# integritychain/fips204

Measured on AMD Instinct MI355X. Metric: ML-DSA-65 verifies/sec per GPU (batched); % HBM roofline, higher is better.
Workload: dtype int32; 1 GPU; ml_dsa_65 batch=65536 whole verify on FIPS 204 wire formats; batch_per_gpu=65536, parallelism=batch-split x1

## Files before the change

### fips204_amd/vfy/vfy.hip

```cpp
#include <hip/hip_runtime.h>
#include <stdint.h>
#include <string.h>

#include <mutex>
#include <string>
#include <vector>

#include "../../include/mldsa_vfy.h"
#include "../layer/layer_dev.h"
#include "../layer/layer_host.h"
#include "../csrc/challenge_dev.h"
#include "../csrc/ntt_wave.h"
#include "../csrc/sampler_dev.h"
#include "../csrc/tables.h"
#include "../csrc/verify_dev.h"
#include "keccak180.h"
#include "vfy_parts.h"

namespace mldsa_vfy {

using mldsa::FWD_TW;
using mldsa::INV_TW;
using mldsa::N;
using mldsa::SHAKE256_RATE;
using mldsa::SWAVES;
using mldsa::Twiddle;
using mldsa::load_le32;
using mldsa::static_for;

#ifndef MLDSA_VFY_EA_WAVES
#define MLDSA_VFY_EA_WAVES 5
#endif
template <int K, int L>
__global__ __launch_bounds__(64 * SWAVES) __attribute__((amdgpu_waves_per_eu(MLDSA_VFY_EA_WAVES, MLDSA_VFY_EA_WAVES))) void k_expand_a(const uint8_t* __restrict__ rho, size_t rho_stride,
                                                                                                    const uint32_t* __restrict__ key_idx,
                                                                                                    int32_t* __restrict__ a_hat, size_t n_ops,
                                                                                                    uint32_t n_keys) {
    const int lane = threadIdx.x & 63;
    const size_t g = (size_t)blockIdx.x * (64 * SWAVES) + threadIdx.x;
    const size_t wave_base = g - lane;
    const size_t n_streams = n_ops * (size_t)(K * L);
    const bool valid = g < n_streams;
    const size_t op = valid ? g / (K * L) : 0;
    const int rs = valid ? (int)(g % (K * L)) : 0;
    const int r = rs / L, sidx = rs % L;
    KeccakState st;
    size_t key = key_idx ? key_idx[op] : op;
    if (n_keys && key >= n_keys) key = 0;
    mldsa::expand_a_seed(st, rho + key * rho_stride, sidx, r);
    rej_ntt_poly_lane_direct180(st, a_hat, wave_base, lane, valid);
}

__global__ __launch_bounds__(256) void k_unpack_a(const uint32_t* __restrict__ packed, int32_t* __restrict__ out, size_t n_polys) {
    const size_t poly = (size_t)blockIdx.x * 4 + (threadIdx.x >> 6);
    if (poly >= n_polys) return;
    const int lane = threadIdx.x & 63;
    const uint32_t* p = packed + poly * mldsa::PACKED_POLY_DWORDS + 3 * lane;
    reinterpret_cast<int4*>(out + poly * N)[lane] = mldsa::unpack24(mldsa::Packed3{p[0], p[1], p[2]});
}

__global__ __launch_bounds__(256) void k_sanitize_keys(const uint32_t* __restrict__ key_idx, uint32_t n_keys, size_t n_ops,
                                                       uint32_t* __restrict__ safe, int32_t* __restrict__ bad) {
    const size_t i = (size_t)blockIdx.x * 256 + threadIdx.x;
    if (i >= n_ops) return;
    const uint32_t k = key_idx[i];
    safe[i] = k < n_keys ? k : 0u;
    bad[i] = k < n_keys ? 0 : 2;
}

constexpr int MU_BLK_STRIDE = 35;
__global__ __launch_bounds__(64) void k_mu(const uint8_t* __restrict__ tr, size_t tr_stride, const uint32_t* __restrict__ key_idx, int mode,
                                           const uint8_t* __restrict__ msgs, const uint64_t* __restrict__ msg_off,
                                           const uint8_t* __restrict__ ctxs, const uint64_t* __restrict__ ctx_off, uint8_t* __restrict__ mu,
                                           size_t mu_stride, int32_t* __restrict__ ctx_bad, const int32_t* __restrict__ key_bad, size_t n_ops,
                                           size_t op0, size_t n_call) {
    __shared__ uint32_t blk[64 * MU_BLK_STRIDE];
    const int lane = threadIdx.x;
    const size_t op = (size_t)blockIdx.x * 64 + lane;
    const bool valid = op < n_ops;
    uint32_t* row = blk + lane * MU_BLK_STRIDE;
    uint8_t* rowb = reinterpret_cast<uint8_t*>(row);

    const uint8_t *trp = nullptr, *mp = nullptr, *cp = nullptr;
    size_t mlen = 0, clen = 0;
    bool live = false;
    if (valid) {
        trp = tr + (key_idx ? key_idx[op] : op) * tr_stride;
        const uint64_t m0 = msg_off[op0 + op], m1 = msg_off[op0 + op + 1];
        bool bad_off = !(msg_off[0] <= m0 && m0 <= m1 && m1 <= msg_off[n_call]);
        mp = msgs + m0;
        mlen = (size_t)(m1 - m0);
        bad_off |= mlen != 0 && msgs == nullptr;
        if (ctx_off) {
            const uint64_t c0 = ctx_off[op0 + op], c1 = ctx_off[op0 + op + 1];
            bad_off |= !(ctx_off[0] <= c0 && c0 <= c1 && c1 <= ctx_off[n_call]);
            cp = ctxs + c0;
            clen = (size_t)(c1 - c0);
            bad_off |= clen != 0 && ctxs == nullptr;
        }
        const int flag = bad_off ? 2 : clen > 255 ? 1 : (key_bad ? key_bad[op] : 0);
        ctx_bad[op] = flag;
        live = !bad_off && clen <= 255;
        if (!live) mlen = clen = 0;
    }
    const size_t pre = (mode == MLDSA_MODE_INTERNAL) ? 0 : 2 + clen;
    const size_t total = live ? 64 + pre + mlen : 0;
    const size_t my_blocks = live ? total / SHAKE256_RATE + 1 : 0;
    size_t max_blocks = my_blocks;
#pragma unroll
    for (int m = 32; m >= 1; m >>= 1) {
        const size_t o = (size_t)__shfl_xor((unsigned long long)max_blocks, m);
        max_blocks = o > max_blocks ? o : max_blocks;
    }
    KeccakState st;
    mldsa::keccak_zero(st);
    for (size_t b = 0; b < max_blocks; b++) {
        if (b < my_blocks) {
            const size_t base = b * SHAKE256_RATE;
            auto byte_at = [&](size_t pos) -> uint8_t {
                if (pos < total) {
                    if (pos < 64) return trp[pos];
                    if (pos < 64 + pre) {
                        const size_t q = pos - 64;
                        return q == 0 ? (uint8_t)(mode == MLDSA_MODE_PREHASH ? 1 : 0) : q == 1 ? (uint8_t)clen : cp[q - 2];
                    }
                    return mp[pos - 64 - pre];
                }
                return pos == total ? (uint8_t)0x1F : (uint8_t)0;
            };
            for (int i = 0; i < SHAKE256_RATE / 4; i++) {
                const size_t pos = base + 4 * (size_t)i;
                uint32_t v;
                if (pos + 4 <= 64) v = load_le32(trp + pos);
                else if (pos >= 64 + pre && pos + 4 <= total) v = load_le32(mp + (pos - 64 - pre));
                else if (pos > total) v = 0;
                else v = (uint32_t)byte_at(pos) | ((uint32_t)byte_at(pos + 1) << 8) | ((uint32_t)byte_at(pos + 2) << 16) | ((uint32_t)byte_at(pos + 3) << 24);
                row[i] = v;
            }
            if (b == my_blocks - 1) rowb[SHAKE256_RATE - 1] |= 0x80;
            static_for<0, 17>([&](auto wc) {
                constexpr int W = decltype(wc)::value;
                st.lo[W] ^= row[2 * W];
                st.hi[W] ^= row[2 * W + 1];
            });
            mldsa::keccak_f1600(st);
        }
    }
    if (valid) {
        uint32_t* out = reinterpret_cast<uint32_t*>(mu + op * mu_stride);
#pragma unroll
        for (int i = 0; i < 8; i++) {
            out[2 * i] = st.lo[i];
            out[2 * i + 1] = st.hi[i];
        }
    }
}

template <int CT>
__global__ __launch_bounds__(64) void k_sample_in_ball(const uint8_t* __restrict__ c_tilde, size_t ct_stride, int tau, uint32_t* __restrict__ c_out,
                                                       size_t n_ops) {
    __shared__ uint32_t c_lds[64 * mldsa::SIB_C_STRIDE];
    __shared__ uint32_t b_lds[64 * mldsa::SIB_BLK_STRIDE];
    const int lane = threadIdx.x;
    const size_t wave_base = (size_t)blockIdx.x * 64;
    const size_t op = wave_base + lane;
    const bool valid = op < n_ops;
    KeccakState st;
    mldsa::keccak_zero(st);
    if (valid) mldsa::absorb_words<CT / 8>(st, c_tilde + op * ct_stride);
    mldsa::shake_pad<SHAKE256_RATE, CT>(st);
    mldsa::sample_in_ball_lane(st, tau, valid, c_lds + lane * mldsa::SIB_C_STRIDE, b_lds + lane * mldsa::SIB_BLK_STRIDE);
    mldsa::wave_lds_sync();
    for (int row = 0; row < 64; row++) {
        if (wave_base + row >= n_ops) break;
        const uint8_t* cb = reinterpret_cast<const uint8_t*>(c_lds + row * mldsa::SIB_C_STRIDE);
        c_out[(wave_base + row) * 64 + lane] =
            (uint32_t)cb[lane] | ((uint32_t)cb[64 + lane] << 8) | ((uint32_t)cb[128 + lane] << 16) | ((uint32_t)cb[192 + lane] << 24);
    }
}

template <int CTRL>
__device__ __forceinline__ int32_t dpp_all(int32_t v) {
    return __builtin_amdgcn_update_dpp(0, v, CTRL, 0xF, 0xF, true);
}

template <int M>
__device__ __forceinline__ void swap_pair(int32_t& x, int32_t& y, int lane) {
    if constexpr (M >= 4) {
        mldsa::swap_pair<M>(x, y, lane);
    } else {
        constexpr int CTRL = M == 2 ? 0x4E : 0xB1;
        const int32_t px = dpp_all<CTRL>(x), py = dpp_all<CTRL>(y);
        const bool up = (lane & M) != 0;
        x = up ? py : x;
        y = up ? y : px;
    }
}
template <int M>
__device__ __forceinline__ void xchg_hi(int32_t r[4], int lane) {
    swap_pair<M>(r[0], r[2], lane);
    swap_pair<M>(r[1], r[3], lane);
}
template <int M>
__device__ __forceinline__ void xchg_lo(int32_t r[4], int lane) {
    swap_pair<M>(r[0], r[1], lane);
    swap_pair<M>(r[2], r[3], lane);
}

template <class TW>
__device__ __forceinline__ void ntt_fwd_wave(int32_t r[4], const TW& tw, int lane) {
    using mldsa::bf_ct;
    bf_ct(r[0], r[2], mldsa::ZF1);
    bf_ct(r[1], r[3], mldsa::ZF1);
    bf_ct(r[0], r[1], mldsa::ZF2);
    bf_ct(r[2], r[3], mldsa::ZF3);
    xchg_hi<32>(r, lane);
    bf_ct(r[0], r[2], tw.get(0));
    bf_ct(r[1], r[3], tw.get(1));
    xchg_lo<16>(r, lane);
    bf_ct(r[0], r[1], tw.get(2));
    bf_ct(r[2], r[3], tw.get(3));
    xchg_hi<8>(r, lane);
    bf_ct(r[0], r[2], tw.get(4));
    bf_ct(r[1], r[3], tw.get(5));
    xchg_lo<4>(r, lane);
    bf_ct(r[0], r[1], tw.get(6));
    bf_ct(r[2], r[3], tw.get(7));
    xchg_hi<2>(r, lane);
    bf_ct(r[0], r[2], tw.get(8));
    bf_ct(r[1], r[3], tw.get(9));
    xchg_lo<1>(r, lane);
    bf_ct(r[0], r[1], tw.get(10));
    bf_ct(r[2], r[3], tw.get(11));
}
template <class TW>
__device__ __forceinline__ void ntt_inv_wave(int32_t r[4], const TW& tw, int lane, int32_t f) {
    using mldsa::bf_gs;
    bf_gs(r[0], r[1], tw.get(0));
    bf_gs(r[2], r[3], tw.get(1));
    bf_gs(r[0], r[2], tw.get(2));
    bf_gs(r[1], r[3], tw.get(3));
    xchg_lo<1>(r, lane);
    bf_gs(r[0], r[1], tw.get(4));
    bf_gs(r[2], r[3], tw.get(5));
    xchg_hi<2>(r, lane);
    bf_gs(r[0], r[2], tw.get(6));
    bf_gs(r[1], r[3], tw.get(7));
    xchg_lo<4>(r, lane);
    bf_gs(r[0], r[1], tw.get(8));
    bf_gs(r[2], r[3], tw.get(9));
    xchg_hi<8>(r, lane);
    bf_gs(r[0], r[2], tw.get(10));
    bf_gs(r[1], r[3], tw.get(11));
    xchg_lo<16>(r, lane);
    bf_gs(r[0], r[1], tw.get(12));
    bf_gs(r[2], r[3], tw.get(13));
    xchg_hi<32>(r, lane);
    const int32_t zf = (int32_t)((((int64_t)mldsa::ZI1 * f) % mldsa::Q) * mldsa::RINV_MOD_Q % mldsa::Q);
#pragma unroll
    for (int k = 0; k < 2; k++) {
        const int32_t a = r[k], b = r[k + 2];
        r[k] = mldsa::caddq(mldsa::mont_mul(a + b, f));
        r[k + 2] = mldsa::caddq(mldsa::mont_mul(a - b, zf));
    }
}

template <bool G2HI>
__device__ __forceinline__ void pack_w1_strided(const uint32_t v[4], uint8_t* dst, int lane) {
    if constexpr (G2HI) {
        uint32_t d[4];
#pragma unroll
        for (int k = 0; k < 4; k++) d[k] = v[k] << (4 * (lane & 7));
#pragma unroll
        for (int k = 0; k < 4; k++) d[k] |= (uint32_t)dpp_all<0xB1>((int32_t)d[k]);
#pragma unroll
        for (int k = 0; k < 4; k++) d[k] |= (uint32_t)dpp_all<0x4E>((int32_t)d[k]);
        const uint32_t d01 = (lane & 1) ? d[1] : d[0], d23 = (lane & 1) ? d[3] : d[2];
        uint32_t mine = (lane & 2) ? d23 : d01;
        mine |= (uint32_t)__builtin_amdgcn_update_dpp(0, (int32_t)mine, 0x104, 0xF, 0xF, true);
        if (!(lane & 4)) mldsa::store_row(reinterpret_cast<uint32_t*>(dst) + 8 * (lane & 3) + (lane >> 3), mine);
    } else {
#pragma unroll
        for (int k = 0; k < 4; k++) {
            const uint32_t n1 = (uint32_t)dpp_all<0xB1>((int32_t)v[k]);
            const uint32_t pair = (lane & 1) ? 0u : (v[k] | (n1 << 6));
            const uint32_t n2 = (uint32_t)dpp_all<0x4E>((int32_t)pair);
            if (!(lane & 3)) {
                const uint32_t q24 = pair | (n2 << 12);
                uint8_t* d = dst + 48 * k + 3 * (lane >> 2);
                d[0] = (uint8_t)q24; d[1] = (uint8_t)(q24 >> 8); d[2] = (uint8_t)(q24 >> 16);
            }
        }
    }
}

constexpr int VW = 4;
template <int K, int L, int GB, bool G2HI, int MINW>
__global__ __launch_bounds__(64 * VW) __attribute__((amdgpu_waves_per_eu(MINW))) void k_verify_main(
    const uint32_t* __restrict__ a_hat, const uint8_t* __restrict__ sigs, size_t sig_len, int ctilde_len, const uint32_t* __restrict__ c,
    const int32_t* __restrict__ t1, const uint32_t* __restrict__ key_idx, size_t key_base, int32_t* __restrict__ hvalid, int omega,
    uint8_t* __restrict__ w1, size_t w1_stride, int32_t* __restrict__ znorm, int32_t zbound, size_t n_ops, const Twiddle* __restrict__ fwd_tab,
    const Twiddle* __restrict__ inv_tab) {
    using mldsa::Packed3;
    constexpr int CB = GB + 1;
    constexpr int BITS = G2HI ? 4 : 6;
    __shared__ int4 zh[VW][L + 1][64];
    __shared__ uint32_t hint_lds[VW][mldsa::HINT_LDS_DWORDS];
    __shared__ Twiddle tw_lds[(FWD_TW + INV_TW) * 64];
    const int lane = threadIdx.x & 63;
    const int wave = __builtin_amdgcn_readfirstlane(threadIdx.x >> 6);
    for (int i = threadIdx.x; i < FWD_TW * 64; i += 64 * VW) tw_lds[i] = fwd_tab[i];
    for (int i = threadIdx.x; i < INV_TW * 64; i += 64 * VW) tw_lds[FWD_TW * 64 + i] = inv_tab[i];
    __syncthreads();
    const mldsa::LdsTw ftw{tw_lds, lane};
    const mldsa::LdsTw itw{tw_lds + FWD_TW * 64, lane};
    const uint32_t wid = blockIdx.x * VW + wave, n_waves = gridDim.x * VW;

    for (size_t op = wid; op < n_ops; op += n_waves) {
        unsigned ul = (unsigned)lane;
        asm volatile("" : "+v"(ul));
        const size_t key = key_idx ? (size_t)__builtin_amdgcn_readfirstlane((int)key_idx[op]) : key_base + op;
        const Packed3* arow = reinterpret_cast<const Packed3*>(a_hat + (op * K * (size_t)L) * mldsa::PACKED_POLY_DWORDS);
        const int4* trow = reinterpret_cast<const int4*>(t1 + (key * K) * (size_t)N);
        Packed3 av[L];
#pragma unroll
        for (int j = 0; j < L; j++) av[j] = mldsa::load_row<mldsa::NT_A_VERIFY>(&arow[(unsigned)(j * 64) + ul]);
        int4 tv = trow[ul];
        const uint8_t* zsrc = sigs + op * sig_len + ctilde_len;
        const mldsa::HintBytes hbytes = mldsa::hint_load(zsrc + L * (32 * CB), omega, K, (int)ul);
        bool zbad = false;
#pragma unroll 1
        for (int j = 0; j <= L; j++) {
            asm volatile("" ::: "memory");
            int32_t r[4];
            if (j < L) {
                const uint8_t* src = zsrc + (size_t)j * (32 * CB);
                int32_t mx = 0;
#pragma unroll
                for (int k = 0; k < 4; k++) {
                    r[k] = mldsa::y_from_raw<CB>(mldsa::y_raw_dword<CB, mldsa::NT_ZC>(src, k, (int)ul), (int)ul);
                    const int32_t a = r[k] < 0 ? -r[k] : r[k];
                    mx = a > mx ? a : mx;
                }
                zbad |= mx >= zbound;
            } else {
                const uint32_t d = mldsa::load_once<mldsa::NT_ZC>(c + op * 64 + ul);
                r[0] = (int8_t)(d & 0xFF); r[1] = (int8_t)((d >> 8) & 0xFF); r[2] = (int8_t)((d >> 16) & 0xFF); r[3] = (int8_t)(d >> 24);
            }
            mldsa_vfy::ntt_fwd_wave(r, ftw, lane);
            if (j == L) {
#pragma unroll
                for (int k = 0; k < 4; k++) r[k] = mldsa::mont_mul(r[k], -1);
            }
            zh[wave][j][lane] = make_int4(r[0], r[1], r[2], r[3]);
        }
        const bool hint_ok = mldsa::hint_unpack_wave<K>(hbytes, omega, hint_lds[wave], (int)ul);
        if (lane == 0) {
            znorm[op] = __ballot(zbad) != 0ull ? 0x7fffffff : 0;
            hvalid[op] = hint_ok ? 1 : 0;
        }
        auto row = [&](int i, const Packed3 (&a_cur)[L], const int4& t_cur, Packed3 (&a_nxt)[L], int4& t_nxt, bool more) {
            const int4 cv = zh[wave][L][lane];
            int64_t acc64[4] = {(int64_t)cv.x * t_cur.x, (int64_t)cv.y * t_cur.y, (int64_t)cv.z * t_cur.z, (int64_t)cv.w * t_cur.w};
#pragma unroll
            for (int j = 0; j < L; j++) {
                const int4 zv = zh[wave][j][lane];
                const int4 a4 = mldsa::unpack24(a_cur[j]);
                acc64[0] += (int64_t)a4.x * zv.x;
                acc64[1] += (int64_t)a4.y * zv.y;
                acc64[2] += (int64_t)a4.z * zv.z;
                acc64[3] += (int64_t)a4.w * zv.w;
            }
            int32_t acc[4];
            if (more) {
#pragma unroll
                for (int j = 0; j < L; j++) a_nxt[j] = mldsa::load_row<mldsa::NT_A_VERIFY>(&arow[(unsigned)(((i + 1) * L + j) * 64) + ul]);
                t_nxt = trow[(unsigned)((i + 1) * 64) + ul];
            }
#pragma unroll
            for (int k = 0; k < 4; k++) acc[k] = mldsa::mont_reduce64(acc64[k]);
            mldsa_vfy::ntt_inv_wave(acc, itw, lane, mldsa::F_MONT2);
            const uint32_t* hrow = hint_lds[wave] + 24 + i * 8 + (ul >> 5);
            uint8_t* dst = w1 + op * w1_stride + (size_t)i * (32 * BITS);
            uint32_t v[4];
#pragma unroll
            for (int k = 0; k < 4; k++) {
                const uint32_t h = (hrow[2 * k] >> (ul & 31)) & 1u;
                v[k] = (uint32_t)mldsa::use_hint<G2HI>((int32_t)h, acc[k]);
            }
            pack_w1_strided<G2HI>(v, dst, lane);
        };
        static_assert(K % 2 == 0, "the row loop runs two rows a trip");
        Packed3 aw[L];
        int4 tw2;
#pragma unroll 1
        for (int i = 0; i < K; i += 2) {
            asm volatile("" ::: "memory");
            row(i, av, tv, aw, tw2, true);
            asm volatile("" ::: "memory");
            row(i + 1, aw, tw2, av, tv, i + 2 < K);
        }
    }
}

constexpr int CWAVES = 4;
constexpr int CBLOCK = 64 * CWAVES;
template <int OUT>
__global__ __launch_bounds__(CBLOCK) void k_ctilde_verdict(const uint8_t* __restrict__ mu_w1, size_t mw, const uint8_t* __restrict__ sigs, size_t sig_len,
                                                           const int32_t* __restrict__ znorm, int32_t zbound, const int32_t* __restrict__ hvalid,
                                                           const int32_t* __restrict__ ctx_bad, uint8_t* __restrict__ ok, size_t n_ops) {
    __shared__ uint32_t tiles[CWAVES * 64 * mldsa::H_STRIDE];
    __shared__ unsigned long long ptr_a[CWAVES * 64];
    const int lane = threadIdx.x & 63, wave = threadIdx.x >> 6;
    uint32_t* tile = tiles + wave * 64 * mldsa::H_STRIDE;
    const size_t base_op = (size_t)blockIdx.x * CBLOCK;
    if (base_op >= n_ops) return;
    const size_t op = base_op + threadIdx.x;
    const bool valid = op < n_ops;
    const size_t opc = valid ? op : base_op;
    ptr_a[wave * 64 + lane] = (unsigned long long)(mu_w1 + opc * mw);
    mldsa::wave_lds_sync_c();
    KeccakState st;
    mldsa::shake256_2_absorb<true>(st, tile, ptr_a + wave * 64, ptr_a + wave * 64, (int)mw, 0, 0, 0, lane);
    if (!valid) return;
    const uint8_t* c0 = sigs + op * sig_len;
    uint32_t diff = 0;
    static_for<0, OUT / 8>([&](auto wc) {
        constexpr int W = decltype(wc)::value;
        diff |= (st.lo[W] ^ load_le32(c0 + 8 * W)) | (st.hi[W] ^ load_le32(c0 + 8 * W + 4));
    });
    ok[op] = (uint8_t)(diff == 0 && znorm[op] < zbound && hvalid[op] && !ctx_bad[op]);
}

}

namespace {

using namespace mldsa_layer;
using namespace mldsa_vfy;

struct DevState {
    int dev = -1;
    int n_cu = 256;
    hipStream_t ea = nullptr, vm = nullptr;
    std::vector<hipEvent_t> ev;
    Twiddle *fwd = nullptr, *inv = nullptr;
    bool prof_on = false;
    std::vector<hipEvent_t> prof_ev;
    std::vector<const char*> prof_name;
    size_t prof_used = 0;
};

std::mutex g_mutex;
std::vector<DevState*> g_states;
size_t g_part_ops = 0;

size_t part_ops() { return g_part_ops ? g_part_ops : (size_t)MLDSA_VFY_PART_OPS; }

int dev_state(const char* fn, int dev, DevState** out) {
    for (DevState* d : g_states)
        if (d->dev == dev) {
            *out = d;
            return MLDSA_OK;
        }
    DevState* d = new DevState;
    d->dev = dev;
    int cu = 0;
    if (hipDeviceGetAttribute(&cu, hipDeviceAttributeMultiprocessorCount, dev) == hipSuccess && cu > 0) d->n_cu = cu;
    const std::vector<mldsa::HostTwiddle> f = mldsa::gen_fwd_lane_twiddles(), i = mldsa::gen_inv_lane_twiddles();
    hipError_t e = hipStreamCreateWithFlags(&d->ea, hipStreamNonBlocking);
    if (e == hipSuccess) e = hipStreamCreateWithFlags(&d->vm, hipStreamNonBlocking);
    if (e == hipSuccess) e = hipMalloc(&d->fwd, f.size() * sizeof(Twiddle));
    if (e == hipSuccess) e = hipMalloc(&d->inv, i.size() * sizeof(Twiddle));
    if (e == hipSuccess) e = hipMemcpy(d->fwd, f.data(), f.size() * sizeof(Twiddle), hipMemcpyHostToDevice);
    if (e == hipSuccess) e = hipMemcpy(d->inv, i.data(), i.size() * sizeof(Twiddle), hipMemcpyHostToDevice);
    if (e != hipSuccess || f.size() != (size_t)FWD_TW * 64 || i.size() != (size_t)INV_TW * 64) {
        if (d->ea) (void)hipStreamDestroy(d->ea);
        if (d->vm) (void)hipStreamDestroy(d->vm);
        if (d->fwd) (void)hipFree(d->fwd);
        if (d->inv) (void)hipFree(d->inv);
        delete d;
        (void)hipGetLastError();
        return e != hipSuccess ? hip_failed(fn, "creating the library's streams and tables", e)
                               : fail(MLDSA_ERR_DEVICE, std::string(fn) + ": the core's twiddle tables have another shape");
    }
    g_states.push_back(d);
    *out = d;
    return MLDSA_OK;
}

struct Events {
    DevState* d;
    size_t used = 0;
    hipError_t err = hipSuccess;
    explicit Events(DevState* d_) : d(d_) {}
    hipEvent_t next() {
        if (used == d->ev.size()) {
            hipEvent_t e = nullptr;
            const hipError_t rc = hipEventCreateWithFlags(&e, hipEventDisableTiming);
            if (rc != hipSuccess) {
                err = rc;
                return nullptr;
            }
            d->ev.push_back(e);
        }
        return d->ev[used++];
    }
};

constexpr size_t PROF_MAX_PAIRS = 4096;
struct ProfScope {
    DevState* d;
    hipStream_t s;
    long idx = -1;
    ProfScope(DevState* d_, hipStream_t s_, const char* name) : d(d_), s(s_) {
        if (!d->prof_on || d->prof_used >= PROF_MAX_PAIRS) return;
        if (d->prof_used * 2 + 2 > d->prof_ev.size()) {
            hipEvent_t a = nullptr, b = nullptr;
            if (hipEventCreate(&a) != hipSuccess) return;
            if (hipEventCreate(&b) != hipSuccess) {
                (void)hipEventDestroy(a);
                return;
            }
            d->prof_ev.push_back(a);
            d->prof_ev.push_back(b);
            d->prof_name.push_back(name);
        } else {
            d->prof_name[d->prof_used] = name;
        }
        idx = (long)d->prof_used++;
        (void)hipEventRecord(d->prof_ev[2 * idx], s);
    }
    ~ProfScope() {
        if (idx >= 0) (void)hipEventRecord(d->prof_ev[2 * idx + 1], s);
    }
};

#define VFY_HIP(call, what)                                     \
    do {                                                        \
        const hipError_t e_ = (call);                           \
        if (e_ != hipSuccess) return hip_failed(fn, what, e_);  \
    } while (0)

#define VFY_BY_SET(set, M)              \
    do {                                \
        if ((set) == MLDSA_44) M(4, 4, 17, false, 32, 5); \
        else if ((set) == MLDSA_65) M(6, 5, 19, true, 48, 4); \
        else M(8, 7, 19, true, 64, 4);  \
    } while (0)

unsigned stream_blocks(size_t n_streams) { return (unsigned)((n_streams + 64 * SWAVES - 1) / (64 * SWAVES)); }

void launch_expand_a(int set, const uint8_t* rho, const uint32_t* key_idx, int32_t* a_hat, size_t n, uint32_t n_keys, hipStream_t s) {
    mldsa_params p;
    (void)mldsa_get_params(set, &p);
    const dim3 grid(stream_blocks(n * (size_t)(p.k * p.l))), block(64 * SWAVES);
#define VFY_EA(KK, LL, GB, G2, CT, MW) hipLaunchKernelGGL((k_expand_a<KK, LL>), grid, block, 0, s, rho, (size_t)32, key_idx, a_hat, n, n_keys)
    VFY_BY_SET(set, VFY_EA);
#undef VFY_EA
}

struct Call {
    int set, mode;
    mldsa_params p;
    const uint8_t *rho, *tr;
    const int32_t* t1;
    size_t n_keys;
    const uint32_t* key_idx;
    const uint8_t* msgs;
    const uint64_t* msg_off;
    const uint8_t* ctxs;
    const uint64_t* ctx_off;
    const uint8_t* sigs;
    uint8_t* ok;
    size_t n_ops;
};

int enqueue(const char* fn, DevState* d, const Call& c, uint8_t* scratch, hipStream_t s) {
    const mldsa_params& p = c.p;
    const PartPlan plan(c.n_ops, part_ops());
    const Carve cv = carve(p.k, p.l, (size_t)p.w1_len, plan);
    const size_t mw = 64 + (size_t)p.w1_len;
    uint32_t* c8 = reinterpret_cast<uint32_t*>(scratch + cv.c);
    int32_t* znorm = reinterpret_cast<int32_t*>(scratch + cv.znorm);
    int32_t* hvalid = reinterpret_cast<int32_t*>(scratch + cv.hvalid);
    int32_t* ctx_bad = reinterpret_cast<int32_t*>(scratch + cv.ctx_bad);
    int32_t* key_bad = reinterpret_cast<int32_t*>(scratch + cv.key_bad);
    uint32_t* kidx = reinterpret_cast<uint32_t*>(scratch + cv.kidx);
    uint8_t* mu_w1 = scratch + cv.mu_w1;
    const size_t sig_len = (size_t)p.sig_len;

    const OrderPlan order = order_plan(plan.n_parts());
    const hipStream_t lanes[N_LANES] = {s, d->ea, d->vm};
    Events evs(d);
    std::vector<hipEvent_t> ev(order.n_events);
    for (hipEvent_t& e : ev) e = evs.next();
    if (evs.err != hipSuccess) return hip_failed(fn, "creating an event", evs.err);

    for (const Step& st : order.steps) {
        const hipStream_t q = lanes[st.lane];
        if (st.act == ACT_RECORD) {
            VFY_HIP(hipEventRecord(ev[st.n], q), (std::string("recording ") + st.what).c_str());
            continue;
        }
        if (st.act == ACT_WAIT) {
            VFY_HIP(hipStreamWaitEvent(q, ev[st.n], 0), (std::string("waiting for ") + st.what).c_str());
            continue;
        }
        const Part part = plan.at(st.n);
        const size_t o = part.first, n = part.count;
        const size_t key_base = c.key_idx ? 0 : o;
        int32_t* a_hat = reinterpret_cast<int32_t*>(scratch + cv.ring[part.half]);
        const uint8_t* sg = c.sigs + o * sig_len;
        const uint32_t* kp = c.key_idx ? kidx + o : nullptr;
        const int32_t* kb = c.key_idx ? key_bad + o : nullptr;
        switch (st.stage) {
        case STAGE_EXPAND_A: {
            ProfScope ps(d, q, "expand_a");
            launch_expand_a(c.set, c.rho + key_base * 32, c.key_idx ? c.key_idx + o : nullptr, a_hat, n, c.key_idx ? (uint32_t)c.n_keys : 0u, q);
            break;
        }
        case STAGE_FRONT: {
            if (c.key_idx)
                hipLaunchKernelGGL(k_sanitize_keys, dim3((unsigned)((n + 255) / 256)), dim3(256), 0, q, c.key_idx + o, (uint32_t)c.n_keys, n, kidx + o, key_bad + o);
            {
                ProfScope ps(d, q, "mu");
                hipLaunchKernelGGL(k_mu, dim3((unsigned)((n + 63) / 64)), dim3(64), 0, q, c.tr + key_base * 64, (size_t)64, kp, c.mode, c.msgs, c.msg_off, c.ctxs,
                                   c.ctx_off, mu_w1 + o * mw, mw, ctx_bad + o, kb, n, o, c.n_ops);
            }
            {
                ProfScope ps(d, q, "sample_in_ball");
                const dim3 grid((unsigned)((n + 63) / 64)), block(64);
#define VFY_SIB(KK, LL, GB, G2, CT, MW) hipLaunchKernelGGL((k_sample_in_ball<CT>), grid, block, 0, q, sg, sig_len, p.tau, c8 + o * 64, n)
                VFY_BY_SET(c.set, VFY_SIB);
#undef VFY_SIB
            }
            break;
        }
        case STAGE_VERIFY_MAIN: {
            ProfScope ps(d, q, "verify_main");
            const size_t need = (n + VW - 1) / VW, cap = (size_t)d->n_cu * 16;
            const dim3 grid((unsigned)(need < cap ? need : cap)), block(64 * VW);
#define VFY_VM(KK, LL, GB, G2, CT, MW)                                                                                                         \
    hipLaunchKernelGGL((k_verify_main<KK, LL, GB, G2, MW>), grid, block, 0, q, reinterpret_cast<const uint32_t*>(a_hat), sg, sig_len,          \
                       p.ctilde_len, c8 + o * 64, c.t1, kp, key_base, hvalid + o, p.omega, mu_w1 + o * mw + 64, mw, znorm + o, p.gamma1 - p.beta, n, \
                       d->fwd, d->inv)
            VFY_BY_SET(c.set, VFY_VM);
#undef VFY_VM
            break;
        }
        default: {
            ProfScope ps(d, q, "ctilde_hash");
            const dim3 grid((unsigned)((n + CBLOCK - 1) / CBLOCK)), block(CBLOCK);
#define VFY_CT(KK, LL, GB, G2, CT, MW)                                                                                                    \
    hipLaunchKernelGGL((k_ctilde_verdict<CT>), grid, block, 0, q, mu_w1 + o * mw, mw, sg, sig_len, znorm + o, p.gamma1 - p.beta, hvalid + o, \
                       ctx_bad + o, c.ok + o, n)
            VFY_BY_SET(c.set, VFY_CT);
#undef VFY_CT
            break;
        }
        }
        LAYER_LAUNCHED(st.what);
    }
    return MLDSA_OK;
}

void drain(DevState* d) {
    (void)hipStreamSynchronize(d->ea);
    (void)hipStreamSynchronize(d->vm);
    (void)hipGetLastError();
}

size_t scratch_bytes_of(int set, size_t n_ops) {
    mldsa_params p;
    if (mldsa_get_params(set, &p) != MLDSA_OK || n_ops > MLDSA_VFY_MAX_OPS) return 0;
    return carve(p.k, p.l, (size_t)p.w1_len, PartPlan(n_ops, part_ops())).bytes;
}

}

extern "C" {

int mldsa_vfy_abi_version(void) { return MLDSA_VFY_ABI_VERSION; }

const char* mldsa_vfy_last_error(void) { return g_err.c_str(); }

size_t mldsa_vfy_scratch_bytes(int set, size_t n_ops) {
    std::lock_guard<std::mutex> lk(g_mutex);
    return scratch_bytes_of(set, n_ops);
}

size_t mldsa_vfy_set_part_ops(size_t part) {
    std::lock_guard<std::mutex> lk(g_mutex);
    const size_t before = part_ops();
    g_part_ops = part;
    return before;
}

int mldsa_vfy_verify(mldsa_ctx* ctx, int set, int mode, const uint8_t* rho, const uint8_t* tr, const int32_t* t1_d2_hat_mont, size_t n_keys,
                     const uint32_t* key_idx, const uint8_t* msgs, const uint64_t* msg_off, const uint8_t* ctxs, const uint64_t* ctx_off,
                     const uint8_t* sigs, uint8_t* ok, size_t n_ops, void* scratch, size_t scratch_bytes, void* stream) {
    const char* fn = "mldsa_vfy_verify";
    Call c;
    const int rc = check_common(fn, ctx, set, n_ops, MLDSA_VFY_MAX_OPS, "MLDSA_VFY_MAX_OPS ops", &c.p);
    if (rc != MLDSA_OK) return rc;
    if (mode != MLDSA_MODE_PURE && mode != MLDSA_MODE_INTERNAL && mode != MLDSA_MODE_PREHASH)
        return fail(MLDSA_ERR_PARAM, std::string(fn) + ": bad mode");
    if (n_ops == 0) return MLDSA_OK;
    if (!rho || !tr || !t1_d2_hat_mont || !msg_off || !sigs || !ok) return fail(MLDSA_ERR_PARAM, std::string(fn) + ": NULL pointer");
    if (key_idx ? n_keys == 0 : n_keys < n_ops) return fail(MLDSA_ERR_PARAM, std::string(fn) + ": n_keys does not cover the batch");
    if (n_keys > 0xFFFFFFFFu) n_keys = 0xFFFFFFFFu;
    if (!aligned(t1_d2_hat_mont, 16)) return fail(MLDSA_ERR_PARAM, std::string(fn) + ": t1_d2_hat_mont must be 16-byte aligned");
    if (!scratch || !aligned(scratch, 256)) return fail(MLDSA_ERR_PARAM, std::string(fn) + ": scratch is NULL or not 256-byte aligned");
    LAYER_ON_DEVICE(ctx);
    std::lock_guard<std::mutex> lk(g_mutex);
    if (scratch_bytes < scratch_bytes_of(set, n_ops))
        return fail(MLDSA_ERR_NOMEM, std::string(fn) + ": scratch is below mldsa_vfy_scratch_bytes(set, n_ops)");
    DevState* d = nullptr;
    const int src = dev_state(fn, dev_, &d);
    if (src != MLDSA_OK) return src;
    c.set = set; c.mode = mode; c.rho = rho; c.tr = tr; c.t1 = t1_d2_hat_mont; c.n_keys = n_keys; c.key_idx = key_idx; c.msgs = msgs;
    c.msg_off = msg_off; c.ctxs = ctxs; c.ctx_off = ctx_off; c.sigs = sigs; c.ok = ok; c.n_ops = n_ops;
    const int erc = enqueue(fn, d, c, static_cast<uint8_t*>(scratch), (hipStream_t)stream);
    if (erc != MLDSA_OK) drain(d);
    return erc;
}

int mldsa_vfy_expand_a(mldsa_ctx* ctx, int set, const uint8_t* rho, int32_t* a_hat, size_t n_ops, void* stream) {
    const char* fn = "mldsa_vfy_expand_a";
    mldsa_params p;
    const int rc = check_common(fn, ctx, set, n_ops, MLDSA_VFY_MAX_OPS, "MLDSA_VFY_MAX_OPS ops", &p);
    if (rc != MLDSA_OK) return rc;
    if (n_ops == 0) return MLDSA_OK;
    if (!rho || !a_hat) return fail(MLDSA_ERR_PARAM, std::string(fn) + ": NULL pointer");
    if (!aligned(a_hat, 16)) return fail(MLDSA_ERR_PARAM, std::string(fn) + ": a_hat must be 16-byte aligned");
    LAYER_ON_DEVICE(ctx);
    hipStream_t s = (hipStream_t)stream;
    const size_t n_polys = n_ops * (size_t)(p.k * p.l);
    void* packed = nullptr;
    VFY_HIP(hipMalloc(&packed, n_polys * PACKED_POLY_BYTES), "allocating the packed rows");
    launch_expand_a(set, rho, nullptr, static_cast<int32_t*>(packed), n_ops, 0u, s);
    hipLaunchKernelGGL(k_unpack_a, dim3((unsigned)((n_polys + 3) / 4)), dim3(256), 0, s, static_cast<const uint32_t*>(packed), a_hat, n_polys);
    hipError_t e = hipGetLastError();
    const hipError_t se = hipStreamSynchronize(s);
    if (e == hipSuccess) e = se;
    (void)hipFree(packed);
    return e == hipSuccess ? MLDSA_OK : hip_failed(fn, "ExpandA and unpack", e);
}

int mldsa_vfy_profile_enable(mldsa_ctx* ctx, int on) {
    const char* fn = "mldsa_vfy_profile_enable";
    if (!ctx) return fail(MLDSA_ERR_PARAM, std::string(fn) + ": NULL context");
    LAYER_ON_DEVICE(ctx);
    std::lock_guard<std::mutex> lk(g_mutex);
    DevState* d = nullptr;
    const int rc = dev_state(fn, dev_, &d);
    if (rc != MLDSA_OK) return rc;
    d->prof_on = on != 0;
    if (!d->prof_on) d->prof_used = 0;
    return MLDSA_OK;
}

int mldsa_vfy_profile_report(mldsa_ctx* ctx, char* buf, size_t buf_len) {
    const char* fn = "mldsa_vfy_profile_report";
    if (!ctx) return fail(MLDSA_ERR_PARAM, std::string(fn) + ": NULL context");
    if (!buf || buf_len <= 2) return fail(MLDSA_ERR_PARAM, std::string(fn) + ": bad argument");
    LAYER_ON_DEVICE(ctx);
    std::lock_guard<std::mutex> lk(g_mutex);
    DevState* d = nullptr;
    const int rc = dev_state(fn, dev_, &d);
    if (rc != MLDSA_OK) return rc;
    VFY_HIP(hipDeviceSynchronize(), "waiting for the device");
    struct Acc { const char* name; double ms; size_t calls; };
    std::vector<Acc> acc;
    for (size_t i = 0; i < d->prof_used; i++) {
        float ms = 0.f;
        if (hipEventElapsedTime(&ms, d->prof_ev[2 * i], d->prof_ev[2 * i + 1]) != hipSuccess) {
            (void)hipGetLastError();
            continue;
        }
        bool found = false;
        for (auto& a : acc)
            if (strcmp(a.name, d->prof_name[i]) == 0) {
                a.ms += ms;
                a.calls++;
                found = true;
                break;
            }
        if (!found) acc.push_back({d->prof_name[i], ms, 1});
    }
    std::string out = "{";
    for (size_t i = 0; i < acc.size(); i++)
        out += std::string(i ? ", " : "") + "\"" + acc[i].name + "\": {\"ms\": " + std::to_string(acc[i].ms) + ", \"calls\": " + std::to_string(acc[i].calls) + "}";
    out += "}";
    if (out.size() + 1 > buf_len) return fail(MLDSA_ERR_PARAM, std::string(fn) + ": buffer too small");
    memcpy(buf, out.c_str(), out.size() + 1);
    d->prof_used = 0;
    return MLDSA_OK;
}

}
```

### fips204_amd/vfy/vfy_parts.h

```cpp
#pragma once
#include <stddef.h>
#include <stdint.h>

#include <vector>

namespace mldsa_vfy {

constexpr size_t PACKED_POLY_BYTES = 768;
constexpr size_t CARVE_ALIGN = 256;

struct Part {
    size_t first = 0, count = 0;
    int half = 0;
};

struct PartPlan {
    size_t n_ops, part;
    PartPlan(size_t n_ops_, size_t part_) : n_ops(n_ops_), part(part_ ? part_ : 1) {}
    size_t n_parts() const { return n_ops / part + (n_ops % part ? 1 : 0); }
    size_t halves() const { return n_parts() > 1 ? 2 : n_parts(); }
    size_t half_ops() const { return n_ops < part ? n_ops : part; }
    Part at(size_t i) const {
        Part p;
        p.first = i * part;
        p.count = n_ops - p.first < part ? n_ops - p.first : part;
        p.half = (int)(i & 1);
        return p;
    }
};

struct Carve {
    size_t ring[2];
    size_t ring_bytes;
    size_t c;
    size_t znorm, hvalid, ctx_bad, key_bad, kidx;
    size_t mu_w1;
    size_t bytes;
};

inline size_t carve_up(size_t x) { return (x + CARVE_ALIGN - 1) / CARVE_ALIGN * CARVE_ALIGN; }

inline Carve carve(int k, int l, size_t w1_len, const PartPlan& plan) {
    Carve c;
    size_t at = 0;
    auto take = [&at](size_t bytes) {
        const size_t here = at;
        at += carve_up(bytes);
        return here;
    };
    c.ring_bytes = plan.half_ops() * (size_t)(k * l) * PACKED_POLY_BYTES;
    c.ring[0] = take(c.ring_bytes);
    c.ring[1] = plan.halves() > 1 ? take(c.ring_bytes) : c.ring[0];
    c.c = take(plan.n_ops * 256);
    c.znorm = take(plan.n_ops * 4);
    c.hvalid = take(plan.n_ops * 4);
    c.ctx_bad = take(plan.n_ops * 4);
    c.key_bad = take(plan.n_ops * 4);
    c.kidx = take(plan.n_ops * 4);
    c.mu_w1 = take(plan.n_ops * (64 + w1_len));
    c.bytes = at + CARVE_ALIGN;
    return c;
}

enum Lane { LANE_CALLER = 0, LANE_EA = 1, LANE_VM = 2, N_LANES = 3 };
enum Action { ACT_RECORD, ACT_WAIT, ACT_LAUNCH };
enum Stage { STAGE_EXPAND_A = 0, STAGE_FRONT = 1, STAGE_VERIFY_MAIN = 2, STAGE_CTILDE = 3, N_STAGES = 4 };

struct Step {
    Lane lane;
    Action act;
    Stage stage;
    size_t n;
    const char* what;
};

struct OrderPlan {
    std::vector<Step> steps;
    size_t n_events = 0;
};

struct StageLanes {
    Lane expand_a, arith, front;
};
inline StageLanes lanes_of_call(size_t n_parts) {
    return n_parts == 1 ? StageLanes{LANE_CALLER, LANE_CALLER, LANE_VM} : StageLanes{LANE_EA, LANE_VM, LANE_CALLER};
}

inline OrderPlan order_plan(size_t n_parts, const StageLanes& on) {
    OrderPlan o;
    if (n_parts == 0) return o;
    const size_t none = (size_t)-1;
    auto put = [&o](Lane lane, Action act, Stage stage, size_t n, const char* what) { o.steps.push_back(Step{lane, act, stage, n, what}); };
    const size_t fork = o.n_events++;
    bool forked[N_LANES] = {true, false, false};
    auto reach = [&](Lane lane, Stage stage) {
        if (!forked[lane]) put(lane, ACT_WAIT, stage, fork, "the fork");
        forked[lane] = true;
    };
    auto record = [&](Lane from, Lane to, Stage stage, const char* what) {
        if (from == to) return none;
        put(from, ACT_RECORD, stage, o.n_events, what);
        return o.n_events++;
    };
    auto wait = [&](Lane to, size_t event, Stage stage, const char* what) {
        if (event == none) return;
        put(to, ACT_WAIT, stage, event, what);
        forked[to] = true;
    };
    put(LANE_CALLER, ACT_RECORD, STAGE_EXPAND_A, fork, "the fork");
    std::vector<size_t> used(n_parts, none);
    for (size_t p = 0; p < n_parts; p++) {
        if (p >= 2) wait(on.expand_a, used[p - 2], STAGE_EXPAND_A, "the ring half");
        reach(on.expand_a, STAGE_EXPAND_A);
        put(on.expand_a, ACT_LAUNCH, STAGE_EXPAND_A, p, "k_expand_a launch");
        const size_t ready = record(on.expand_a, on.arith, STAGE_EXPAND_A, "ExpandA's end");
        reach(on.front, STAGE_FRONT);
        put(on.front, ACT_LAUNCH, STAGE_FRONT, p, "front launch");
        const size_t front = record(on.front, on.arith, STAGE_FRONT, "the front's end");
        wait(on.arith, ready, STAGE_EXPAND_A, "ExpandA");
        wait(on.arith, front, STAGE_FRONT, "the front");
        reach(on.arith, STAGE_VERIFY_MAIN);
        put(on.arith, ACT_LAUNCH, STAGE_VERIFY_MAIN, p, "k_verify_main launch");
        if (p + 2 < n_parts) used[p] = record(on.arith, on.expand_a, STAGE_VERIFY_MAIN, "the end of the ring half's use");
        put(on.arith, ACT_LAUNCH, STAGE_CTILDE, p, "k_ctilde_verdict launch");
    }
    wait(LANE_CALLER, record(on.arith, LANE_CALLER, STAGE_CTILDE, "the join"), STAGE_CTILDE, "the join");
    return o;
}

inline OrderPlan order_plan(size_t n_parts) { return order_plan(n_parts, lanes_of_call(n_parts)); }

}
```

Measured before the change: 41.16 million verifies/s.

## Batch forward NTTs of z and c across lane groups with register butterflies

Replaces the serial per-polynomial forward NTT loop (one poly per wave pass, 4 coefficients per lane) with passes that process 4 or 2 polynomials at once. Each lane holds 16 or 8 coefficients, so the early NTT levels run as in-register butterflies with compile-time zetas and only the later levels use cross-lane swaps and a 256-entry zeta table. The LDS row is padded to 65 entries to avoid bank conflicts on the new store pattern, and the forward twiddle table is loaded only when a leftover single pass still needs it. The intent is fewer cross-lane exchanges and fewer serialized passes per op, at the cost of higher register pressure and more code, which may reduce occupancy.

Result: no change. 41.33 million verifies/s, median of 6 (+0.4%).

```diff
diff --git a/fips204_amd/vfy/vfy.hip b/fips204_amd/vfy/vfy.hip
--- a/fips204_amd/vfy/vfy.hip
+++ b/fips204_amd/vfy/vfy.hip
@@ -265,6 +265,78 @@
     }
 }
 
+constexpr int ZH_ROW = 65;
+template <int P>
+constexpr FwdPlan FWD_PLAN = fwd_plan(P);
+template <int P, int J0, int CB, int L>
+__device__ __forceinline__ bool fwd_pass(const uint8_t* zsrc, const uint32_t* c_op, int4 (*zw)[ZH_ROW], const Twiddle* zt, int32_t zbound, unsigned ul) {
+    using mldsa::bf_ct;
+    constexpr int R = 4 * P, W = 64 / P;
+    static_assert(J0 + P <= L + 1 && (W * CB) % 8 == 0, "the slots are polynomials of the op; a register's fields start at whole bytes");
+    constexpr bool HAS_C = J0 + P == L + 1;
+    constexpr int LP = FWD_PLAN<P>.lp, RB = FWD_PLAN<P>.rb;
+    const unsigned p = ul & (P - 1), l = ul >> LP;
+    const bool is_c = HAS_C && p == P - 1;
+    int32_t r[R];
+    bool zbad = false;
+    if (!is_c) {
+        const uint8_t* src = zsrc + (size_t)(J0 + p) * (32 * CB);
+        int32_t mx = 0;
+#pragma unroll
+        for (int k = 0; k < R; k++) {
+            r[k] = mldsa::y_from_raw<CB>(mldsa::y_raw_dword<CB, mldsa::NT_ZC>(src + k * (W * CB / 8), 0, (int)l), (int)l);
+            const int32_t a = r[k] < 0 ? -r[k] : r[k];
+            mx = a > mx ? a : mx;
+        }
+        zbad = mx >= zbound;
+    } else {
+        uint32_t d[P];
+#pragma unroll
+        for (int q = 0; q < P; q++) d[q] = mldsa::load_once<mldsa::NT_ZC>(c_op + W * q + l);
+#pragma unroll
+        for (int k = 0; k < R; k++) r[k] = (int8_t)((d[k % P] >> (8 * (k / P))) & 0xFF);
+    }
+    static_for<0, FWD_PLAN<P>.n_in>([&](auto ic) {
+        constexpr int I = decltype(ic)::value, BIT = 1 << (RB - 1 - I);
+        static_for<0, (1 << I)>([&](auto gc) {
+            constexpr int G0 = decltype(gc)::value * 2 * BIT;
+            constexpr int32_t Z = zeta_mont(fwd_in_zeta(FWD_PLAN<P>, I, G0));
+            int32_t z = Z;
+            asm volatile("" : "+s"(z));
+#pragma unroll
+            for (int k = G0; k < G0 + BIT; k++) bf_ct(r[k], r[k + BIT], z);
+        });
+    });
+    static_for<0, FWD_PLAN<P>.n_x>([&](auto ic) {
+        constexpr int I = decltype(ic)::value, BIT = 1 << FWD_PLAN<P>.x[I].reg_bit, M = FWD_PLAN<P>.x[I].mask;
+        asm volatile("" ::: "memory");
+        const Twiddle* zl = zt + ((ul >> (LP + FWD_PLAN<P>.x[I].s)) << (RB - 1));
+        static_for<0, R>([&](auto kc) {
+            constexpr int K0 = decltype(kc)::value;
+            if constexpr (!(K0 & BIT)) mldsa_vfy::swap_pair<M>(r[K0], r[K0 | BIT], (int)ul);
+        });
+        static_for<0, R>([&](auto kc) {
+            constexpr int K0 = decltype(kc)::value;
+            if constexpr (!(K0 & BIT)) {
+                constexpr int ZR = fwd_x_zeta_reg(FWD_PLAN<P>, I, K0);
+                bf_ct(r[K0], r[K0 | BIT], zl[ZR]);
+            }
+        });
+    });
+    if (is_c) {
+#pragma unroll
+        for (int k = 0; k < R; k++) r[k] = mldsa::mont_mul(r[k], -1);
+    }
+    int4* dst = zw[J0 + p] + (l << (RB - 2));
+    static_for<0, R / 4>([&](auto qc) {
+        constexpr int Q4 = 4 * decltype(qc)::value;
+        constexpr int A = fwd_last_reg(FWD_PLAN<P>, Q4), B = fwd_last_reg(FWD_PLAN<P>, Q4 + 1), C = fwd_last_reg(FWD_PLAN<P>, Q4 + 2),
+                      D = fwd_last_reg(FWD_PLAN<P>, Q4 + 3);
+        dst[Q4 / 4] = make_int4(r[A], r[B], r[C], r[D]);
+    });
+    return zbad;
+}
+
 template <bool G2HI>
 __device__ __forceinline__ void pack_w1_strided(const uint32_t v[4], uint8_t* dst, int lane) {
     if constexpr (G2HI) {
@@ -300,20 +372,24 @@
     const uint32_t* __restrict__ a_hat, const uint8_t* __restrict__ sigs, size_t sig_len, int ctilde_len, const uint32_t* __restrict__ c,
     const int32_t* __restrict__ t1, const uint32_t* __restrict__ key_idx, size_t key_base, int32_t* __restrict__ hvalid, int omega,
     uint8_t* __restrict__ w1, size_t w1_stride, int32_t* __restrict__ znorm, int32_t zbound, size_t n_ops, const Twiddle* __restrict__ fwd_tab,
-    const Twiddle* __restrict__ inv_tab) {
+    const Twiddle* __restrict__ inv_tab, const Twiddle* __restrict__ zeta_tab) {
     using mldsa::Packed3;
     constexpr int CB = GB + 1;
     constexpr int BITS = G2HI ? 4 : 6;
-    __shared__ int4 zh[VW][L + 1][64];
+    constexpr int QUADS = (L + 1) / 4, REST = (L + 1) % 4;
+    static_assert(QUADS >= 1 && QUADS <= 2 && REST <= 2, "the passes below");
+    constexpr int TW_ZETA = INV_TW * 64, TW_FWD = TW_ZETA + 256;
+    __shared__ int4 zh[VW][L + 1][ZH_ROW];
     __shared__ uint32_t hint_lds[VW][mldsa::HINT_LDS_DWORDS];
-    __shared__ Twiddle tw_lds[(FWD_TW + INV_TW) * 64];
+    __shared__ Twiddle tw_lds[TW_FWD + (REST == 1 ? FWD_TW * 64 : 0)];
     const int lane = threadIdx.x & 63;
     const int wave = __builtin_amdgcn_readfirstlane(threadIdx.x >> 6);
-    for (int i = threadIdx.x; i < FWD_TW * 64; i += 64 * VW) tw_lds[i] = fwd_tab[i];
-    for (int i = threadIdx.x; i < INV_TW * 64; i += 64 * VW) tw_lds[FWD_TW * 64 + i] = inv_tab[i];
+    for (int i = threadIdx.x; i < INV_TW * 64; i += 64 * VW) tw_lds[i] = inv_tab[i];
+    for (int i = threadIdx.x; i < 256; i += 64 * VW) tw_lds[TW_ZETA + i] = zeta_tab[i];
+    if constexpr (REST == 1)
+        for (int i = threadIdx.x; i < FWD_TW * 64; i += 64 * VW) tw_lds[TW_FWD + i] = fwd_tab[i];
     __syncthreads();
-    const mldsa::LdsTw ftw{tw_lds, lane};
-    const mldsa::LdsTw itw{tw_lds + FWD_TW * 64, lane};
+    const mldsa::LdsTw itw{tw_lds, lane};
     const uint32_t wid = blockIdx.x * VW + wave, n_waves = gridDim.x * VW;
 
     for (size_t op = wid; op < n_ops; op += n_waves) {
@@ -328,32 +404,23 @@
         int4 tv = trow[ul];
         const uint8_t* zsrc = sigs + op * sig_len + ctilde_len;
         const mldsa::HintBytes hbytes = mldsa::hint_load(zsrc + L * (32 * CB), omega, K, (int)ul);
-        bool zbad = false;
-#pragma unroll 1
-        for (int j = 0; j <= L; j++) {
+        const uint32_t* c_op = c + op * 64;
+        const Twiddle* zt = tw_lds + TW_ZETA;
+        mldsa::wave_lds_sync();
+        bool zbad = fwd_pass<4, 0, CB, L>(zsrc, c_op, zh[wave], zt, zbound, ul);
+        if constexpr (QUADS == 2) zbad |= fwd_pass<4, 4, CB, L>(zsrc, c_op, zh[wave], zt, zbound, ul);
+        if constexpr (REST == 2) zbad |= fwd_pass<2, 4 * QUADS, CB, L>(zsrc, c_op, zh[wave], zt, zbound, ul);
+        if constexpr (REST == 1) {
             asm volatile("" ::: "memory");
-            int32_t r[4];
-            if (j < L) {
-                const uint8_t* src = zsrc + (size_t)j * (32 * CB);
-                int32_t mx = 0;
-#pragma unroll
-                for (int k = 0; k < 4; k++) {
-                    r[k] = mldsa::y_from_raw<CB>(mldsa::y_raw_dword<CB, mldsa::NT_ZC>(src, k, (int)ul), (int)ul);
-                    const int32_t a = r[k] < 0 ? -r[k] : r[k];
-                    mx = a > mx ? a : mx;
-                }
-                zbad |= mx >= zbound;
-            } else {
-                const uint32_t d = mldsa::load_once<mldsa::NT_ZC>(c + op * 64 + ul);
-                r[0] = (int8_t)(d & 0xFF); r[1] = (int8_t)((d >> 8) & 0xFF); r[2] = (int8_t)((d >> 16) & 0xFF); r[3] = (int8_t)(d >> 24);
-            }
+            const mldsa::LdsTw ftw{tw_lds + TW_FWD, lane};
+            const uint32_t d = mldsa::load_once<mldsa::NT_ZC>(c_op + ul);
+            int32_t r[4] = {(int8_t)(d & 0xFF), (int8_t)((d >> 8) & 0xFF), (int8_t)((d >> 16) & 0xFF), (int8_t)(d >> 24)};
             mldsa_vfy::ntt_fwd_wave(r, ftw, lane);
-            if (j == L) {
-#pragma unroll
-                for (int k = 0; k < 4; k++) r[k] = mldsa::mont_mul(r[k], -1);
-            }
-            zh[wave][j][lane] = make_int4(r[0], r[1], r[2], r[3]);
-        }
+#pragma unroll
+            for (int k = 0; k < 4; k++) r[k] = mldsa::mont_mul(r[k], -1);
+            zh[wave][L][lane] = make_int4(r[0], r[1], r[2], r[3]);
+        }
+        mldsa::wave_lds_sync();
         const bool hint_ok = mldsa::hint_unpack_wave<K>(hbytes, omega, hint_lds[wave], (int)ul);
         if (lane == 0) {
             znorm[op] = __ballot(zbad) != 0ull ? 0x7fffffff : 0;
@@ -444,7 +511,7 @@
     int n_cu = 256;
     hipStream_t ea = nullptr, vm = nullptr;
     std::vector<hipEvent_t> ev;
-    Twiddle *fwd = nullptr, *inv = nullptr;
+    Twiddle *fwd = nullptr, *inv = nullptr, *zeta = nullptr;
     bool prof_on = false;
     std::vector<hipEvent_t> prof_ev;
     std::vector<const char*> prof_name;
@@ -468,17 +535,22 @@
     int cu = 0;
     if (hipDeviceGetAttribute(&cu, hipDeviceAttributeMultiprocessorCount, dev) == hipSuccess && cu > 0) d->n_cu = cu;
     const std::vector<mldsa::HostTwiddle> f = mldsa::gen_fwd_lane_twiddles(), i = mldsa::gen_inv_lane_twiddles();
+    int32_t z[256];
+    mldsa::gen_zeta_table_mont(z);
     hipError_t e = hipStreamCreateWithFlags(&d->ea, hipStreamNonBlocking);
     if (e == hipSuccess) e = hipStreamCreateWithFlags(&d->vm, hipStreamNonBlocking);
     if (e == hipSuccess) e = hipMalloc(&d->fwd, f.size() * sizeof(Twiddle));
     if (e == hipSuccess) e = hipMalloc(&d->inv, i.size() * sizeof(Twiddle));
+    if (e == hipSuccess) e = hipMalloc(&d->zeta, sizeof(z));
     if (e == hipSuccess) e = hipMemcpy(d->fwd, f.data(), f.size() * sizeof(Twiddle), hipMemcpyHostToDevice);
     if (e == hipSuccess) e = hipMemcpy(d->inv, i.data(), i.size() * sizeof(Twiddle), hipMemcpyHostToDevice);
+    if (e == hipSuccess) e = hipMemcpy(d->zeta, z, sizeof(z), hipMemcpyHostToDevice);
     if (e != hipSuccess || f.size() != (size_t)FWD_TW * 64 || i.size() != (size_t)INV_TW * 64) {
         if (d->ea) (void)hipStreamDestroy(d->ea);
         if (d->vm) (void)hipStreamDestroy(d->vm);
         if (d->fwd) (void)hipFree(d->fwd);
         if (d->inv) (void)hipFree(d->inv);
+        if (d->zeta) (void)hipFree(d->zeta);
         delete d;
         (void)hipGetLastError();
         return e != hipSuccess ? hip_failed(fn, "creating the library's streams and tables", e)
@@ -644,7 +716,7 @@
 #define VFY_VM(KK, LL, GB, G2, CT, MW)                                                                                                         \
     hipLaunchKernelGGL((k_verify_main<KK, LL, GB, G2, MW>), grid, block, 0, q, reinterpret_cast<const uint32_t*>(a_hat), sg, sig_len,          \
                        p.ctilde_len, c8 + o * 64, c.t1, kp, key_base, hvalid + o, p.omega, mu_w1 + o * mw + 64, mw, znorm + o, p.gamma1 - p.beta, n, \
-                       d->fwd, d->inv)
+                       d->fwd, d->inv, d->zeta)
             VFY_BY_SET(c.set, VFY_VM);
 #undef VFY_VM
             break;
diff --git a/fips204_amd/vfy/vfy_parts.h b/fips204_amd/vfy/vfy_parts.h
--- a/fips204_amd/vfy/vfy_parts.h
+++ b/fips204_amd/vfy/vfy_parts.h
@@ -130,4 +130,71 @@
 
 inline OrderPlan order_plan(size_t n_parts) { return order_plan(n_parts, lanes_of_call(n_parts)); }
 
-}
+constexpr int32_t FWD_Q = 8380417;
+
+constexpr int32_t zeta_mont(int m) {
+    int e = 0;
+    for (int b = 0; b < 8; b++) e |= ((m >> b) & 1) << (7 - b);
+    int64_t x = 1;
+    for (int i = 0; i < e; i++) x = x * 1753 % FWD_Q;
+    return (int32_t)((x << 32) % FWD_Q);
+}
+
+struct FwdLevel {
+    int s;
+    int mask;
+    int reg_bit;
+    int reg_coef[4];
+};
+
+struct FwdPlan {
+    int p, lp, rb, regs;
+    int n_in;
+    int n_x;
+    FwdLevel x[5];
+    int reg_coef[4];
+};
+
+constexpr FwdPlan fwd_plan(int P) {
+    FwdPlan f{};
+    f.p = P;
+    f.lp = P == 4 ? 2 : 1;
+    f.rb = f.lp + 2;
+    f.regs = 4 * P;
+    f.n_in = f.rb;
+    f.n_x = 8 - f.rb;
+    int held[4] = {0, 0, 0, 0};
+    for (int t = 0; t < f.rb; t++) held[t] = 8 - f.rb + t;
+    for (int i = 0; i < f.n_x; i++) {
+        FwdLevel& x = f.x[i];
+        x.s = 7 - f.rb - i;
+        x.mask = 1 << (f.lp + x.s);
+        x.reg_bit = 0;
+        for (int t = 0; t < f.rb; t++)
+            if (held[t] == x.s + f.rb) x.reg_bit = t;
+        held[x.reg_bit] = x.s;
+        for (int t = 0; t < 4; t++) x.reg_coef[t] = held[t];
+    }
+    for (int t = 0; t < 4; t++) f.reg_coef[t] = held[t];
+    return f;
+}
+
+constexpr int fwd_slot(const FwdPlan& f, int lane) { return lane & (f.p - 1); }
+constexpr int fwd_first_coef(const FwdPlan& f, int lane, int reg) { return (64 / f.p) * reg + (lane >> f.lp); }
+constexpr int fwd_in_zeta(const FwdPlan& f, int i, int reg) { return (1 << i) + (reg >> (f.rb - i)); }
+constexpr int fwd_x_zeta_reg(const FwdPlan& f, int i, int reg) {
+    const FwdLevel& x = f.x[i];
+    int m = 128 >> x.s;
+    for (int t = 0; t < f.rb; t++)
+        if (t != x.reg_bit) m += ((reg >> t) & 1) << (x.reg_coef[t] - x.s - 1);
+    return m;
+}
+constexpr int fwd_x_zeta_lane(const FwdPlan& f, int i, int lane) { return (lane >> (f.lp + f.x[i].s)) << (f.rb - 1); }
+constexpr int fwd_last_base(const FwdPlan& f, int lane) { return (lane >> f.lp) << f.rb; }
+constexpr int fwd_last_reg(const FwdPlan& f, int at) {
+    int reg = 0;
+    for (int t = 0; t < f.rb; t++) reg |= ((at >> f.reg_coef[t]) & 1) << t;
+    return reg;
+}
+
+}
```
